# raulmur/ORB_SLAM2

Measured on NVIDIA H100. Metric: stereo frames/sec (ORB extract L+R + ComputeStereoMatches, KITTI-shaped 1242x375 @2000 kpts), higher is better.
Workload: dtype u8

## Files before the change

### orb_slam2_b200/csrc/borb_internal.h

```cpp
#pragma once
#include <cuda_runtime.h>
#include <stdint.h>

#include <mutex>
#include <string>
#include <vector>

#include "../../include/borb.h"

namespace borb {

constexpr int EDGE = 19;
constexpr int PATCH = 31;
constexpr int HALF_PATCH = 15;
constexpr int MIN_BORDER = 16;
constexpr int TH_HIGH = 100;
constexpr int TH_LOW = 50;
constexpr int BLUR_TILE_W = 120;
constexpr int BLUR_TILE_H = 64;
constexpr int FAST_TILE_W = 124;
constexpr int FAST_H_BAND = 64;

__host__ __device__ inline int fast_rows_per_blk(int nRows, int hCell) {
    const int r = FAST_H_BAND / hCell;
    return r < 1 ? 1 : (r > nRows ? nRows : r);
}
__host__ __device__ inline int fast_box_rows(int rowsPerBlk, int hCell) { return rowsPerBlk * hCell + 6; }

__host__ __device__ inline uint32_t pack_xys(int x, int y, int s) { return (uint32_t)x | ((uint32_t)y << 12) | ((uint32_t)s << 24); }
__host__ __device__ inline int xys_x(uint32_t v) { return (int)(v & 0xFFFu); }
__host__ __device__ inline int xys_y(uint32_t v) { return (int)((v >> 12) & 0xFFFu); }
__host__ __device__ inline int xys_s(uint32_t v) { return (int)(v >> 24); }

struct LevelGeom {
    int w, h;
    int pitch;
    unsigned pyr_off;
    int nCols, nRows, wCell, hCell;
    int cellsPerBlk;
    int rowsPerBlk;
    int blkCols;
    int blkBase;
    unsigned cand_off;
    int cand_cap;
    int quota;
    int nIni;
    float hX;
    int node_cap;
    int sel_off;
    float scale;
    float inv_scale;
    float patch_size;
    unsigned xtab_off, ytab_off;
    unsigned xwin_off;
    int x_windowed;
};

struct Geometry {
    int nlevels;
    int w, h;
    int ini_th, min_th;
    int fast_mode;
    int fast_blocks;
    unsigned pyr_image_stride;
    unsigned cand_image_stride;
    int sel_image_stride;
    int blur_tiles;
    int blur_base[BORB_MAX_LEVELS + 1];
    int umax[16];
    LevelGeom lv[BORB_MAX_LEVELS];
};

struct Workspace {
    int max_images = 0;
    uint8_t* pyr = nullptr;
    uint8_t* blur = nullptr;
    uint32_t* cand = nullptr;
    int* cand_cnt = nullptr;
    int* pnode = nullptr;
    uint32_t* sel = nullptr;
    int* sel_cnt = nullptr;
    borb_keypoint* kps = nullptr;
    uint8_t* desc = nullptr;
    int* nkp = nullptr;
    float* u_right = nullptr;
    float* depth = nullptr;
    int* sad = nullptr;
    int16_t* tabs = nullptr;
    uint32_t* brief_slots = nullptr;
    int* pair_idx = nullptr;
    int* st_bins = nullptr;
    void* st_recs = nullptr;
    uint8_t* stage = nullptr;
    size_t stage_bytes = 0;
    void* fast_tmaps = nullptr;
    void* fast_tiles = nullptr;
    int fast_n_tiles = 0;
};

constexpr int BRIEF_BINS = 32;
const std::vector<uint32_t>& brief_slot_table();

void set_error(const char* fmt, ...);
bool allow_max_smem(const void* func);
#define BORB_CUDA(call)                                                                             \
    do {                                                                                            \
        cudaError_t _e = (call);                                                                    \
        if (_e != cudaSuccess) {                                                                    \
            borb::set_error("%s failed: %s (%s:%d)", #call, cudaGetErrorString(_e), __FILE__, __LINE__); \
            return (_e == cudaErrorNoDevice || _e == cudaErrorInsufficientDriver) ? BORB_ERR_NO_DEVICE : BORB_ERR_CUDA; \
        }                                                                                           \
    } while (0)

int launch_repack_remap(const Geometry& g, const Workspace& ws, const uint8_t* stage, int src_stride, size_t src_image_bytes, int src_w,
                        int src_h, const float* mx0, const float* my0, const float* mx1, const float* my1, int n_images, cudaStream_t s);
int launch_repack_color(const Geometry& g, const Workspace& ws, const uint8_t* stage, int src_stride, size_t src_image_bytes, int channels,
                        int rgb, int n_images, cudaStream_t s);
int launch_repack(const Geometry& g, const Workspace& ws, const uint8_t* stage, int src_stride, size_t src_image_bytes,
                  int n_images, cudaStream_t s);
int launch_pyramid(const Geometry& g, const Workspace& ws, int n_images, cudaStream_t s);
int launch_fast(const Geometry& g, const Workspace& ws, int n_images, cudaStream_t s);
int launch_quadtree(const Geometry& g, const Workspace& ws, int n_images, cudaStream_t s);
int launch_blur(const Geometry& g, const Workspace& ws, int n_images, cudaStream_t s);
int launch_describe(const Geometry& g, const Workspace& ws, int n_images, cudaStream_t s);

struct StereoView {
    const uint8_t* pyr;
    const borb_keypoint* kps;
    const uint8_t* desc;
    const int* nkp;
    unsigned pyr_image_stride;
    int kp_image_stride;
};
int launch_stereo(const Geometry& g, const StereoView& L, const StereoView& R, const int* d_pair_idx, int n_pairs,
                  float bf, float b, float* d_u_right, float* d_depth, int* d_sad, int out_stride, int* d_bins, void* d_recs,
                  cudaStream_t s);
int stereo_rec_stride(const Geometry& g);
size_t stereo_bins_bytes_per_pair();
size_t stereo_rec_bytes();
size_t quadtree_smem_bytes(int node_cap);
borb_status build_fast_tmaps(const Geometry& g, const Workspace& ws, void* out_tmaps);
borb_status build_fast_tiles(const Geometry& g, Workspace& ws);
size_t fast_tmaps_bytes();

}

struct borb_extractor {
    borb_extractor_cfg cfg;
    int device = 0;
    cudaStream_t stream = nullptr;
    std::vector<float> scale, inv_scale, sigma2, inv_sigma2;
    std::vector<int> per_level;
    int umax[16];
    bool have_geom = false;
    borb::Geometry geom;
    borb::Workspace ws;
    int last_n_images = 0;
    int last_stereo_pairs = 0;
    int in_channels = 1;
    int in_rgb = 1;
    float* d_map[2][2] = {{nullptr, nullptr}, {nullptr, nullptr}};
    int map_src_w = 0, map_src_h = 0, map_dst_w = 0, map_dst_h = 0;
    int fast_mode = 0;
    uint64_t launches = 0;
    static constexpr int EV_RING = 128;
    bool timing = false;
    std::vector<cudaEvent_t> ev;
    unsigned ev_mask[EV_RING] = {};
    int ev_slot = 0;
    int ev_pending = 0;
    float stage_ms[8] = {};
    double stage_sum_ms[8] = {};
    uint64_t stage_steps = 0;
    int* h_counts = nullptr;
    std::vector<int> pair_cache;
};
```

### orb_slam2_b200/csrc/k_blur.cu

```cuda
#include "borb_internal.h"

namespace borb {

namespace {
constexpr int BT_R = 16;
constexpr int BT_WARPS = BLUR_TILE_H / BT_R;

__device__ __forceinline__ int reflect101(int p, int len) {
    if (p < 0) p = -p;
    if (p >= len) p = 2 * len - 2 - p;
    return min(max(p, 0), len - 1);
}
}

__global__ void __launch_bounds__(32 * BT_WARPS) blur_kernel(const __grid_constant__ Geometry g, const uint8_t* __restrict__ pyr,
                                                             uint8_t* __restrict__ blur) {
    const int img = blockIdx.y;
    int l = 0;
    while (l + 1 < g.nlevels && (int)blockIdx.x >= g.blur_base[l + 1]) l++;
    const LevelGeom& L = g.lv[l];
    const int local = blockIdx.x - g.blur_base[l];
    const int tilesX = (L.w + BLUR_TILE_W - 1) / BLUR_TILE_W;
    const int ty = local / tilesX, tx = local - ty * tilesX;
    const int lane = threadIdx.x & 31, wrp = threadIdx.x >> 5;
    const int x = tx * BLUR_TILE_W + 4 * (lane - 1);
    const int yb = ty * BLUR_TILE_H + wrp * BT_R;
    if (yb >= L.h) return;
    const uint8_t* src = pyr + (size_t)img * g.pyr_image_stride + L.pyr_off;
    uint8_t* dst = blur + (size_t)img * g.pyr_image_stride + L.pyr_off;
    const int W = L.w, H = L.h, pitch = L.pitch;
    const bool left_edge = (x == 0);
    const bool loads = x >= 0 && x < pitch;
    const bool stores = lane >= 1 && lane <= 30 && x < W;
    const unsigned WLO = 18u | (34u << 8) | (48u << 16) | (56u << 24);
    const unsigned WHI = 48u | (34u << 8) | (18u << 16);

    uint32_t own[BT_R + 6];
    if (yb >= 3 && yb + BT_R + 2 < H) {
        const uint8_t* p = src + (size_t)(yb - 3) * pitch + x;
#pragma unroll
        for (int step = 0; step < BT_R + 6; step++, p += pitch) own[step] = loads ? *reinterpret_cast<const uint32_t*>(p) : 0u;
    } else {
#pragma unroll
        for (int step = 0; step < BT_R + 6; step++)
            own[step] = loads ? *reinterpret_cast<const uint32_t*>(src + (unsigned)(reflect101(yb + step - 3, H) * pitch) + x) : 0u;
    }

    uint32_t pk[6][4];
    uint32_t hprev[4] = {0, 0, 0, 0};
#pragma unroll
    for (int step = 0; step < BT_R + 6; step++) {
        const uint32_t W1 = own[step];
        uint32_t W0 = __shfl_up_sync(0xFFFFFFFFu, W1, 1);
        const uint32_t W2 = __shfl_down_sync(0xFFFFFFFFu, W1, 1);
        if (left_edge) W0 = __byte_perm(W1, W2, 0x1234);
        uint32_t h[4];
        h[0] = __dp4a(__byte_perm(W0, W1, 0x4321), WLO, __dp4a(__byte_perm(W1, W2, 0x4321), WHI, 0u));
        h[1] = __dp4a(__byte_perm(W0, W1, 0x5432), WLO, __dp4a(__byte_perm(W1, W2, 0x5432), WHI, 0u));
        h[2] = __dp4a(__byte_perm(W0, W1, 0x6543), WLO, __dp4a(__byte_perm(W1, W2, 0x6543), WHI, 0u));
        h[3] = __dp4a(W1, WLO, __dp4a(W2, WHI, 0u));
        if (step >= 1) {
#pragma unroll
            for (int i = 0; i < 4; i++) pk[(step - 1) % 6][i] = __byte_perm(hprev[i], h[i], 0x5410);
        }
        if (step >= 6) {
            const int yout = yb + step - 6;
            if (yout < H && stores) {
                uint32_t s[4];
#pragma unroll
                for (int i = 0; i < 4; i++) {
                    uint32_t acc = h[i] * 18u + 32768u;
                    acc = __dp2a_lo(pk[(step - 2) % 6][i], 48u | (34u << 8), acc);
                    acc = __dp2a_lo(pk[(step - 4) % 6][i], 48u | (56u << 8), acc);
                    s[i] = __dp2a_lo(pk[(step - 6) % 6][i], 18u | (34u << 8), acc);
                }
                const uint32_t out = __byte_perm(__byte_perm(s[0], s[1], 0x0062), __byte_perm(s[2], s[3], 0x0062), 0x5410);
                *reinterpret_cast<uint32_t*>(dst + (size_t)yout * pitch + x) = out;
            }
        }
#pragma unroll
        for (int i = 0; i < 4; i++) hprev[i] = h[i];
    }
}

int launch_blur(const Geometry& g, const Workspace& ws, int n_images, cudaStream_t s) {
    dim3 grid(g.blur_tiles, n_images);
    blur_kernel<<<grid, 32 * BT_WARPS, 0, s>>>(g, ws.pyr, ws.blur);
    return 1;
}

}
```

### orb_slam2_b200/csrc/k_pyramid.cu

```cuda
#include "borb_internal.h"

namespace borb {

template <int ROWS>
__global__ void __launch_bounds__(256, 6) pyr_resize_kernel(const uint8_t* __restrict__ pyr, uint8_t* __restrict__ pyr_out,
                                                         const int16_t* __restrict__ tabs, LevelGeom src, LevelGeom dst,
                                                         unsigned image_stride) {
    const int img = blockIdx.z;
    const int dyb = (blockIdx.y * 8 + threadIdx.y) * ROWS;
    const int dx0 = (blockIdx.x * 32 + threadIdx.x) * 4;
    const int wpad = (dst.w + 8 + 3) & ~3;
    if (dyb >= dst.h || dx0 >= wpad) return;
    const uint8_t* S = pyr + (size_t)img * image_stride + src.pyr_off;
    uint8_t* D = pyr_out + (size_t)img * image_stride + dst.pyr_off;
    const uint4* xt = reinterpret_cast<const uint4*>(tabs + ((size_t)dst.xwin_off + dx0) * 4);
    const uint2* yt = reinterpret_cast<const uint2*>(tabs + (size_t)dst.ytab_off * 4);
    const uint4 e01 = xt[0], e23 = xt[1];
    const uint32_t wts[4] = {e01.x, e01.z, e23.x, e23.z};
    const uint32_t ctl[4] = {e01.y, e01.w, e23.y, e23.w};
    const int base = (int)(ctl[0] & 0xFFFF);
    uint32_t ra[ROWS][3], rc[ROWS][3];
    uint32_t B0[ROWS], B1[ROWS];
#pragma unroll
    for (int r = 0; r < ROWS; r++) {
        const int dy = min(dyb + r, dst.h - 1);
        const uint2 ye = yt[dy];
        const int sy = (int)(short)(ye.x & 0xFFFF);
        B0[r] = ye.x & 0xFFFF0000u;
        B1[r] = ye.y << 16;
        const int sy0 = min(max(sy, 0), src.h - 1), sy1 = min(max(sy + 1, 0), src.h - 1);
        const uint32_t* R0 = reinterpret_cast<const uint32_t*>(S + (size_t)sy0 * src.pitch + base);
        const uint32_t* R1 = reinterpret_cast<const uint32_t*>(S + (size_t)sy1 * src.pitch + base);
        ra[r][0] = R0[0]; ra[r][1] = R0[1]; ra[r][2] = R0[2];
        rc[r][0] = R1[0]; rc[r][1] = R1[1]; rc[r][2] = R1[2];
    }
#pragma unroll
    for (int r = 0; r < ROWS; r++) {
        if (dyb + r >= dst.h) break;
        uint32_t v[4];
#pragma unroll
        for (int i = 0; i < 4; i++) {
            const uint32_t s1 = ctl[i] >> 16, s2 = ctl[i] >> 24;
            const uint32_t p0 = __byte_perm(__byte_perm(ra[r][0], ra[r][1], s1), ra[r][2], s2);
            const uint32_t p1 = __byte_perm(__byte_perm(rc[r][0], rc[r][1], s1), rc[r][2], s2);
            const uint32_t h0 = __dp2a_lo(wts[i], p0, 0u), h1 = __dp2a_lo(wts[i], p1, 0u);
            v[i] = (__umulhi(B0[r], h0 >> 4) + __umulhi(B1[r], h1 >> 4) + 2) >> 2;
        }
        const uint32_t out = __byte_perm(__byte_perm(v[0], v[1], 0x0040), __byte_perm(v[2], v[3], 0x0040), 0x5410);
        *reinterpret_cast<uint32_t*>(D + (size_t)(dyb + r) * dst.pitch + dx0) = out;
    }
}

__global__ void __launch_bounds__(256) pyr_resize_generic_kernel(const uint8_t* __restrict__ pyr, uint8_t* __restrict__ pyr_out,
                                                                 const int16_t* __restrict__ tabs, LevelGeom src, LevelGeom dst,
                                                                 unsigned image_stride) {
    const int img = blockIdx.z;
    const int dy = blockIdx.y * 8 + threadIdx.y;
    const int dx = blockIdx.x * 32 + threadIdx.x;
    const int wpad = (dst.w + 8 + 3) & ~3;
    if (dy >= dst.h || dx >= wpad) return;
    const uint8_t* S = pyr + (size_t)img * image_stride + src.pyr_off;
    uint8_t* D = pyr_out + (size_t)img * image_stride + dst.pyr_off;
    const short4 xe = reinterpret_cast<const short4*>(tabs)[(size_t)dst.xtab_off + dx];
    const short4 ye = reinterpret_cast<const short4*>(tabs)[(size_t)dst.ytab_off + dy];
    const int sy0 = min(max((int)ye.x, 0), src.h - 1), sy1 = min(max((int)ye.x + 1, 0), src.h - 1);
    const uint8_t* R0 = S + (size_t)sy0 * src.pitch;
    const uint8_t* R1 = S + (size_t)sy1 * src.pitch;
    const int sx = xe.x;
    const int r0 = R0[sx] * xe.y + R0[sx + 1] * xe.z;
    const int r1 = R1[sx] * xe.y + R1[sx + 1] * xe.z;
    D[(size_t)dy * dst.pitch + dx] = (uint8_t)((((ye.y * (r0 >> 4)) >> 16) + ((ye.z * (r1 >> 4)) >> 16) + 2) >> 2);
}

__global__ void __launch_bounds__(256) repack_kernel(const uint8_t* __restrict__ stage, int src_stride, size_t src_image_bytes,
                                                     uint8_t* __restrict__ pyr, LevelGeom l0, unsigned image_stride) {
    const int img = blockIdx.z, y = blockIdx.y;
    const int x0 = (blockIdx.x * 256 + threadIdx.x) * 4;
    if (x0 >= l0.w) return;
    const uint8_t* S = stage + (size_t)img * src_image_bytes + (size_t)y * src_stride + x0;
    uint32_t v = 0;
#pragma unroll
    for (int i = 0; i < 4; i++)
        if (x0 + i < l0.w) v |= (uint32_t)S[i] << (8 * i);
    *reinterpret_cast<uint32_t*>(pyr + (size_t)img * image_stride + l0.pyr_off + (size_t)y * l0.pitch + x0) = v;
}

__global__ void __launch_bounds__(256) repack_color_kernel(const uint8_t* __restrict__ stage, int src_stride, size_t src_image_bytes,
                                                           int channels, int rgb, uint8_t* __restrict__ pyr, LevelGeom l0,
                                                           unsigned image_stride) {
    const int img = blockIdx.z, y = blockIdx.y;
    const int x0 = (blockIdx.x * 256 + threadIdx.x) * 4;
    if (x0 >= l0.w) return;
    const uint8_t* S = stage + (size_t)img * src_image_bytes + (size_t)y * src_stride + (size_t)x0 * channels;
    const int cr = rgb ? 9798 : 3735, cb = rgb ? 3735 : 9798;
    uint32_t v = 0;
#pragma unroll
    for (int i = 0; i < 4; i++)
        if (x0 + i < l0.w) {
            const uint8_t* px = S + i * channels;
            const int yv = (px[0] * cr + px[1] * 19235 + px[2] * cb + 16384) >> 15;
            v |= (uint32_t)yv << (8 * i);
        }
    *reinterpret_cast<uint32_t*>(pyr + (size_t)img * image_stride + l0.pyr_off + (size_t)y * l0.pitch + x0) = v;
}

__global__ void __launch_bounds__(256) repack_remap_kernel(const uint8_t* __restrict__ stage, int src_stride, size_t src_image_bytes,
                                                           int src_w, int src_h, const float* __restrict__ mx0,
                                                           const float* __restrict__ my0, const float* __restrict__ mx1,
                                                           const float* __restrict__ my1, uint8_t* __restrict__ pyr, LevelGeom l0,
                                                           unsigned image_stride) {
    const int img = blockIdx.z, y = blockIdx.y;
    const int x0 = (blockIdx.x * 256 + threadIdx.x) * 4;
    if (x0 >= l0.w) return;
    const bool second = (img & 1) && mx1 != nullptr;
    const float* MX = second ? mx1 : mx0;
    const float* MY = second ? my1 : my0;
    const uint8_t* S = stage + (size_t)img * src_image_bytes;
    uint32_t v = 0;
#pragma unroll
    for (int i = 0; i < 4; i++)
        if (x0 + i < l0.w) {
            const size_t o = (size_t)y * l0.w + x0 + i;
            const int sx = __float2int_rn(__fmul_rn(MX[o], 32.f)), sy = __float2int_rn(__fmul_rn(MY[o], 32.f));
            const int ix = max(-32768, min(32767, sx >> 5)), iy = max(-32768, min(32767, sy >> 5));
            const int fx = sx & 31, fy = sy & 31;
            auto tap = [&](int yy, int xx) -> int {
                return (xx >= 0 && xx < src_w && yy >= 0 && yy < src_h) ? (int)S[(size_t)yy * src_stride + xx] : 0;
            };
            const int w00 = (32 - fx) * (32 - fy) * 32, w01 = fx * (32 - fy) * 32, w10 = (32 - fx) * fy * 32, w11 = fx * fy * 32;
            const int r = (tap(iy, ix) * w00 + tap(iy, ix + 1) * w01 + tap(iy + 1, ix) * w10 + tap(iy + 1, ix + 1) * w11 + 16384) >> 15;
            v |= (uint32_t)r << (8 * i);
        }
    *reinterpret_cast<uint32_t*>(pyr + (size_t)img * image_stride + l0.pyr_off + (size_t)y * l0.pitch + x0) = v;
}

__global__ void __launch_bounds__(256) pad_level0_kernel(uint8_t* __restrict__ pyr, LevelGeom l0, unsigned image_stride) {
    const int y = blockIdx.x * 256 + threadIdx.x, img = blockIdx.y;
    if (y >= l0.h) return;
    uint8_t* row = pyr + (size_t)img * image_stride + l0.pyr_off + (size_t)y * l0.pitch;
#pragma unroll
    for (int k = 0; k < 8; k++) row[l0.w + k] = row[max(l0.w - 2 - k, 0)];
}

int launch_repack(const Geometry& g, const Workspace& ws, const uint8_t* stage, int src_stride, size_t src_image_bytes,
                  int n_images, cudaStream_t s) {
    dim3 grid((g.lv[0].w + 1023) / 1024, g.lv[0].h, n_images);
    repack_kernel<<<grid, 256, 0, s>>>(stage, src_stride, src_image_bytes, ws.pyr, g.lv[0], g.pyr_image_stride);
    return 1;
}

constexpr int PYR_ROWS = 2;

int launch_repack_remap(const Geometry& g, const Workspace& ws, const uint8_t* stage, int src_stride, size_t src_image_bytes, int src_w,
                        int src_h, const float* mx0, const float* my0, const float* mx1, const float* my1, int n_images, cudaStream_t s) {
    dim3 grid((g.lv[0].w + 1023) / 1024, g.lv[0].h, n_images);
    repack_remap_kernel<<<grid, 256, 0, s>>>(stage, src_stride, src_image_bytes, src_w, src_h, mx0, my0, mx1, my1, ws.pyr, g.lv[0],
                                             g.pyr_image_stride);
    return 1;
}

int launch_repack_color(const Geometry& g, const Workspace& ws, const uint8_t* stage, int src_stride, size_t src_image_bytes, int channels,
                        int rgb, int n_images, cudaStream_t s) {
    dim3 grid((g.lv[0].w + 1023) / 1024, g.lv[0].h, n_images);
    repack_color_kernel<<<grid, 256, 0, s>>>(stage, src_stride, src_image_bytes, channels, rgb, ws.pyr, g.lv[0], g.pyr_image_stride);
    return 1;
}

int launch_pyramid(const Geometry& g, const Workspace& ws, int n_images, cudaStream_t s) {
    int launches = 0;
    pad_level0_kernel<<<dim3((g.lv[0].h + 255) / 256, n_images), 256, 0, s>>>(ws.pyr, g.lv[0], g.pyr_image_stride);
    launches++;
    for (int l = 1; l < g.nlevels; l++) {
        const LevelGeom& d = g.lv[l];
        dim3 block(32, 8);
        if (d.x_windowed) {
            dim3 grid((d.w + 8 + 127) / 128, (d.h + 8 * PYR_ROWS - 1) / (8 * PYR_ROWS), n_images);
            pyr_resize_kernel<PYR_ROWS><<<grid, block, 0, s>>>(ws.pyr, ws.pyr, ws.tabs, g.lv[l - 1], d, g.pyr_image_stride);
        } else {
            dim3 grid((d.w + 8 + 3 + 31) / 32, (d.h + 7) / 8, n_images);
            pyr_resize_generic_kernel<<<grid, block, 0, s>>>(ws.pyr, ws.pyr, ws.tabs, g.lv[l - 1], d, g.pyr_image_stride);
        }
        launches++;
    }
    return launches;
}

}
```

Baseline: 44040.

## Widen blur tiles to 8 pixels per lane and reuse shared source rows in pyramid resize

The Gaussian blur kernel now has each lane handle 8 pixels instead of 4. Tiles become 256 wide, so the redundant halo lanes go away; lane 0 and lane 31 load the edge bytes themselves. Row loads are pipelined through an 8-deep register prefetch ring, and two output rows are produced per pair of input steps. The pyramid resize kernel processes 4 rows per thread, skips reloading a source row when it equals the previous row's lower row, and reuses that row's horizontal result; its launch-bounds minimum-blocks hint drops from 6 to 4. The changes aim to cut wasted loads and ALU work, at the cost of higher register pressure and lower occupancy.

```diff
diff --git a/orb_slam2_b200/csrc/borb_internal.h b/orb_slam2_b200/csrc/borb_internal.h
--- a/orb_slam2_b200/csrc/borb_internal.h
+++ b/orb_slam2_b200/csrc/borb_internal.h
@@ -16,7 +16,7 @@
 constexpr int MIN_BORDER = 16;
 constexpr int TH_HIGH = 100;
 constexpr int TH_LOW = 50;
-constexpr int BLUR_TILE_W = 120;
+constexpr int BLUR_TILE_W = 256;
 constexpr int BLUR_TILE_H = 64;
 constexpr int FAST_TILE_W = 124;
 constexpr int FAST_H_BAND = 64;
diff --git a/orb_slam2_b200/csrc/k_blur.cu b/orb_slam2_b200/csrc/k_blur.cu
--- a/orb_slam2_b200/csrc/k_blur.cu
+++ b/orb_slam2_b200/csrc/k_blur.cu
@@ -5,11 +5,27 @@
 namespace {
 constexpr int BT_R = 16;
 constexpr int BT_WARPS = BLUR_TILE_H / BT_R;
+constexpr int BT_STEPS = BT_R + 6;
+constexpr int BT_PF = 8;
+static_assert(BLUR_TILE_W == 32 * 8 && BT_R % 2 == 0 && BLUR_TILE_H % BT_R == 0, "blur tiling");
 
 __device__ __forceinline__ int reflect101(int p, int len) {
     if (p < 0) p = -p;
     if (p >= len) p = 2 * len - 2 - p;
     return min(max(p, 0), len - 1);
+}
+
+__device__ __forceinline__ void row_pass4(uint32_t W0, uint32_t W1, uint32_t W2, uint32_t* h) {
+    const unsigned WLO = 18u | (34u << 8) | (48u << 16) | (56u << 24);
+    const unsigned WHI = 48u | (34u << 8) | (18u << 16);
+    h[0] = __dp4a(__byte_perm(W0, W1, 0x4321), WLO, __dp4a(__byte_perm(W1, W2, 0x4321), WHI, 0u));
+    h[1] = __dp4a(__byte_perm(W0, W1, 0x5432), WLO, __dp4a(__byte_perm(W1, W2, 0x5432), WHI, 0u));
+    h[2] = __dp4a(__byte_perm(W0, W1, 0x6543), WLO, __dp4a(__byte_perm(W1, W2, 0x6543), WHI, 0u));
+    h[3] = __dp4a(W1, WLO, __dp4a(W2, WHI, 0u));
+}
+
+__device__ __forceinline__ uint32_t pack_out(const uint32_t* s) {
+    return __byte_perm(__byte_perm(s[0], s[1], 0x0062), __byte_perm(s[2], s[3], 0x0062), 0x5410);
 }
 }
 
@@ -23,63 +39,68 @@
     const int tilesX = (L.w + BLUR_TILE_W - 1) / BLUR_TILE_W;
     const int ty = local / tilesX, tx = local - ty * tilesX;
     const int lane = threadIdx.x & 31, wrp = threadIdx.x >> 5;
-    const int x = tx * BLUR_TILE_W + 4 * (lane - 1);
+    const int x = tx * BLUR_TILE_W + 8 * lane;
     const int yb = ty * BLUR_TILE_H + wrp * BT_R;
     if (yb >= L.h) return;
     const uint8_t* src = pyr + (size_t)img * g.pyr_image_stride + L.pyr_off;
     uint8_t* dst = blur + (size_t)img * g.pyr_image_stride + L.pyr_off;
     const int W = L.w, H = L.h, pitch = L.pitch;
-    const bool left_edge = (x == 0);
-    const bool loads = x >= 0 && x < pitch;
-    const bool stores = lane >= 1 && lane <= 30 && x < W;
-    const unsigned WLO = 18u | (34u << 8) | (48u << 16) | (56u << 24);
-    const unsigned WHI = 48u | (34u << 8) | (18u << 16);
+    const bool loads = x < pitch;
+    const bool stores = x < W;
+    const int xe = lane == 0 ? x - 4 : x + 8;
+    const bool ext = (lane == 0 && x > 0) || (lane == 31 && xe < pitch);
 
-    uint32_t own[BT_R + 6];
-    if (yb >= 3 && yb + BT_R + 2 < H) {
-        const uint8_t* p = src + (size_t)(yb - 3) * pitch + x;
+    uint2 buf[BT_PF];
+    uint32_t ebuf[BT_PF];
+    auto load = [&](int step, int slot) {
+        const uint8_t* row = src + (unsigned)(reflect101(yb + step - 3, H) * pitch);
+        buf[slot] = loads ? *reinterpret_cast<const uint2*>(row + x) : make_uint2(0u, 0u);
+        ebuf[slot] = ext ? *reinterpret_cast<const uint32_t*>(row + xe) : 0u;
+    };
 #pragma unroll
-        for (int step = 0; step < BT_R + 6; step++, p += pitch) own[step] = loads ? *reinterpret_cast<const uint32_t*>(p) : 0u;
-    } else {
+    for (int step = 0; step < BT_PF; step++) load(step, step);
+
+    uint32_t P[4][8];
+    uint32_t heven[8];
 #pragma unroll
-        for (int step = 0; step < BT_R + 6; step++)
-            own[step] = loads ? *reinterpret_cast<const uint32_t*>(src + (unsigned)(reflect101(yb + step - 3, H) * pitch) + x) : 0u;
-    }
-
-    uint32_t pk[6][4];
-    uint32_t hprev[4] = {0, 0, 0, 0};
+    for (int step = 0; step < BT_STEPS; step++) {
+        if (step >= 8 && (step & 1) == 0 && yb + step - 6 >= H) break;
+        const uint32_t a = buf[step % BT_PF].x, b = buf[step % BT_PF].y, e = ebuf[step % BT_PF];
+        if (step + BT_PF < BT_STEPS) load(step + BT_PF, step % BT_PF);
+        uint32_t left = __shfl_up_sync(0xFFFFFFFFu, b, 1);
+        uint32_t right = __shfl_down_sync(0xFFFFFFFFu, a, 1);
+        if (lane == 0) left = x == 0 ? __byte_perm(a, b, 0x1234) : e;
+        if (lane == 31) right = e;
+        uint32_t h[8];
+        row_pass4(left, a, b, h);
+        row_pass4(a, b, right, h + 4);
+        if ((step & 1) == 0) {
 #pragma unroll
-    for (int step = 0; step < BT_R + 6; step++) {
-        const uint32_t W1 = own[step];
-        uint32_t W0 = __shfl_up_sync(0xFFFFFFFFu, W1, 1);
-        const uint32_t W2 = __shfl_down_sync(0xFFFFFFFFu, W1, 1);
-        if (left_edge) W0 = __byte_perm(W1, W2, 0x1234);
-        uint32_t h[4];
-        h[0] = __dp4a(__byte_perm(W0, W1, 0x4321), WLO, __dp4a(__byte_perm(W1, W2, 0x4321), WHI, 0u));
-        h[1] = __dp4a(__byte_perm(W0, W1, 0x5432), WLO, __dp4a(__byte_perm(W1, W2, 0x5432), WHI, 0u));
-        h[2] = __dp4a(__byte_perm(W0, W1, 0x6543), WLO, __dp4a(__byte_perm(W1, W2, 0x6543), WHI, 0u));
-        h[3] = __dp4a(W1, WLO, __dp4a(W2, WHI, 0u));
-        if (step >= 1) {
+            for (int i = 0; i < 8; i++) heven[i] = h[i];
+            continue;
+        }
+        const int k = step >> 1;
 #pragma unroll
-            for (int i = 0; i < 4; i++) pk[(step - 1) % 6][i] = __byte_perm(hprev[i], h[i], 0x5410);
+        for (int i = 0; i < 8; i++) P[k % 4][i] = __byte_perm(heven[i], h[i], 0x5410);
+        if (k < 3) continue;
+        const int m = k - 3;
+        const int y0 = yb + 2 * m;
+        uint32_t s0[8], s1[8];
+#pragma unroll
+        for (int i = 0; i < 8; i++) {
+            uint32_t acc = heven[i] * 18u + 32768u;
+            acc = __dp2a_lo(P[(m + 2) % 4][i], 48u | (34u << 8), acc);
+            acc = __dp2a_lo(P[(m + 1) % 4][i], 48u | (56u << 8), acc);
+            s0[i] = __dp2a_lo(P[m % 4][i], 18u | (34u << 8), acc);
+            acc = __dp2a_lo(P[k % 4][i], 34u | (18u << 8), 32768u);
+            acc = __dp2a_lo(P[(m + 2) % 4][i], 56u | (48u << 8), acc);
+            acc = __dp2a_lo(P[(m + 1) % 4][i], 34u | (48u << 8), acc);
+            s1[i] = __dp2a_lo(P[m % 4][i], 18u << 8, acc);
         }
-        if (step >= 6) {
-            const int yout = yb + step - 6;
-            if (yout < H && stores) {
-                uint32_t s[4];
-#pragma unroll
-                for (int i = 0; i < 4; i++) {
-                    uint32_t acc = h[i] * 18u + 32768u;
-                    acc = __dp2a_lo(pk[(step - 2) % 6][i], 48u | (34u << 8), acc);
-                    acc = __dp2a_lo(pk[(step - 4) % 6][i], 48u | (56u << 8), acc);
-                    s[i] = __dp2a_lo(pk[(step - 6) % 6][i], 18u | (34u << 8), acc);
-                }
-                const uint32_t out = __byte_perm(__byte_perm(s[0], s[1], 0x0062), __byte_perm(s[2], s[3], 0x0062), 0x5410);
-                *reinterpret_cast<uint32_t*>(dst + (size_t)yout * pitch + x) = out;
-            }
+        if (stores) {
+            *reinterpret_cast<uint2*>(dst + (size_t)y0 * pitch + x) = make_uint2(pack_out(s0), pack_out(s0 + 4));
+            if (y0 + 1 < H) *reinterpret_cast<uint2*>(dst + (size_t)(y0 + 1) * pitch + x) = make_uint2(pack_out(s1), pack_out(s1 + 4));
         }
-#pragma unroll
-        for (int i = 0; i < 4; i++) hprev[i] = h[i];
     }
 }
 
diff --git a/orb_slam2_b200/csrc/k_pyramid.cu b/orb_slam2_b200/csrc/k_pyramid.cu
--- a/orb_slam2_b200/csrc/k_pyramid.cu
+++ b/orb_slam2_b200/csrc/k_pyramid.cu
@@ -3,7 +3,7 @@
 namespace borb {
 
 template <int ROWS>
-__global__ void __launch_bounds__(256, 6) pyr_resize_kernel(const uint8_t* __restrict__ pyr, uint8_t* __restrict__ pyr_out,
+__global__ void __launch_bounds__(256, 4) pyr_resize_kernel(const uint8_t* __restrict__ pyr, uint8_t* __restrict__ pyr_out,
                                                          const int16_t* __restrict__ tabs, LevelGeom src, LevelGeom dst,
                                                          unsigned image_stride) {
     const int img = blockIdx.z;
@@ -21,6 +21,8 @@
     const int base = (int)(ctl[0] & 0xFFFF);
     uint32_t ra[ROWS][3], rc[ROWS][3];
     uint32_t B0[ROWS], B1[ROWS];
+    bool fresh[ROWS];
+    int prev_sy1 = -1;
 #pragma unroll
     for (int r = 0; r < ROWS; r++) {
         const int dy = min(dyb + r, dst.h - 1);
@@ -29,23 +31,32 @@
         B0[r] = ye.x & 0xFFFF0000u;
         B1[r] = ye.y << 16;
         const int sy0 = min(max(sy, 0), src.h - 1), sy1 = min(max(sy + 1, 0), src.h - 1);
-        const uint32_t* R0 = reinterpret_cast<const uint32_t*>(S + (size_t)sy0 * src.pitch + base);
+        fresh[r] = sy0 != prev_sy1;
+        prev_sy1 = sy1;
+        if (fresh[r]) {
+            const uint32_t* R0 = reinterpret_cast<const uint32_t*>(S + (size_t)sy0 * src.pitch + base);
+            ra[r][0] = R0[0]; ra[r][1] = R0[1]; ra[r][2] = R0[2];
+        }
         const uint32_t* R1 = reinterpret_cast<const uint32_t*>(S + (size_t)sy1 * src.pitch + base);
-        ra[r][0] = R0[0]; ra[r][1] = R0[1]; ra[r][2] = R0[2];
         rc[r][0] = R1[0]; rc[r][1] = R1[1]; rc[r][2] = R1[2];
     }
+    uint32_t s1[4], s2[4];
+#pragma unroll
+    for (int i = 0; i < 4; i++) { s1[i] = ctl[i] >> 16; s2[i] = ctl[i] >> 24; }
+    uint32_t q1[4] = {0, 0, 0, 0};
 #pragma unroll
     for (int r = 0; r < ROWS; r++) {
         if (dyb + r >= dst.h) break;
+        uint32_t q0[4];
+#pragma unroll
+        for (int i = 0; i < 4; i++) {
+            if (fresh[r]) q0[i] = __dp2a_lo(wts[i], __byte_perm(__byte_perm(ra[r][0], ra[r][1], s1[i]), ra[r][2], s2[i]), 0u) >> 4;
+            else q0[i] = q1[i];
+            q1[i] = __dp2a_lo(wts[i], __byte_perm(__byte_perm(rc[r][0], rc[r][1], s1[i]), rc[r][2], s2[i]), 0u) >> 4;
+        }
         uint32_t v[4];
 #pragma unroll
-        for (int i = 0; i < 4; i++) {
-            const uint32_t s1 = ctl[i] >> 16, s2 = ctl[i] >> 24;
-            const uint32_t p0 = __byte_perm(__byte_perm(ra[r][0], ra[r][1], s1), ra[r][2], s2);
-            const uint32_t p1 = __byte_perm(__byte_perm(rc[r][0], rc[r][1], s1), rc[r][2], s2);
-            const uint32_t h0 = __dp2a_lo(wts[i], p0, 0u), h1 = __dp2a_lo(wts[i], p1, 0u);
-            v[i] = (__umulhi(B0[r], h0 >> 4) + __umulhi(B1[r], h1 >> 4) + 2) >> 2;
-        }
+        for (int i = 0; i < 4; i++) v[i] = (__umulhi(B0[r], q0[i]) + __umulhi(B1[r], q1[i]) + 2) >> 2;
         const uint32_t out = __byte_perm(__byte_perm(v[0], v[1], 0x0040), __byte_perm(v[2], v[3], 0x0040), 0x5410);
         *reinterpret_cast<uint32_t*>(D + (size_t)(dyb + r) * dst.pitch + dx0) = out;
     }
@@ -149,7 +160,7 @@
     return 1;
 }
 
-constexpr int PYR_ROWS = 2;
+constexpr int PYR_ROWS = 4;
 
 int launch_repack_remap(const Geometry& g, const Workspace& ws, const uint8_t* stage, int src_stride, size_t src_image_bytes, int src_w,
                         int src_h, const float* mx0, const float* my0, const float* mx1, const float* my1, int n_images, cudaStream_t s) {
```

Result: faster. 45280, median of 6 (+2.8%).
